# kornelski/cavif-rs

Hardware: AMD Instinct MI355X
Metric: MPix/s encoded at speed=4 q=80, 1080p batch; bit-exact vs CPU oracle (higher is better)
Workload: dtype u16 samples / i32 transform / i64 RD cost

## Files before the change

### cavif_rs_amd/csrc/dev_group.h

```cpp
#pragma once
#include "dev_predict.h"
#include "dev_txfm.h"
#include "dev_rate.h"

struct GroupBuf8 {
  int32_t tbuf[8 * 9];
  int32_t cbuf[64];
  int32_t qc[64];
  uint16_t rec[64];
  uint8_t lev[144];
};
#define GROUP_LANE (LANE & 15)
#define GROUP_ID (LANE >> 4)

template <int CTRL> __device__ __forceinline__ int dpp_row_(int v) { return __builtin_amdgcn_update_dpp(0, v, CTRL, 0xF, 0xF, false); }
__device__ __forceinline__ int row_sum_i32(int v) { v += dpp_row_<0x128>(v); v += dpp_row_<0x124>(v); v += dpp_row_<0x122>(v); v += dpp_row_<0x121>(v); return v; }
__device__ __forceinline__ int row_max_i32(int v) {
  v = imax_(v, dpp_row_<0x128>(v)); v = imax_(v, dpp_row_<0x124>(v)); v = imax_(v, dpp_row_<0x122>(v)); v = imax_(v, dpp_row_<0x121>(v)); return v;
}

static __device__ const int tx4_tab[2][3][4][8] = {
  { { { 2896, 2896, 2896, 2896, 0, 0, 0, 0 }, { 3784, 1567, -1567, -3784, 0, 0, 0, 0 }, { 2896, -2896, -2896, 2896, 0, 0, 0, 0 }, { 1567, -3784, 3784, -1567, 0, 0, 0, 0 } },
    { { 1321, 2482, 3344, 3803, 0, 0, 0, 0 }, { 3344, 3344, 0, -3344, 0, 0, 0, 0 }, { 3803, -1321, -3344, 2482, 0, 0, 0, 0 }, { 2482, -3803, 3344, -1321, 0, 0, 0, 0 } },
    { { 5793, 0, 0, 0, 0, 0, 0, 0 }, { 0, 5793, 0, 0, 0, 0, 0, 0 }, { 0, 0, 5793, 0, 0, 0, 0, 0 }, { 0, 0, 0, 5793, 0, 0, 0, 0 } } },
// ... 163 lines not shown
    int32_t x[N];
#pragma unroll
    for (int r = 0; r < N; r++) x[r] = (int32_t)((uint32_t)gb->tbuf[r * P + gl] << 2);
    tx1d<N>(x, ck, true);
#pragma unroll
    for (int r = 0; r < N; r++) gb->tbuf[r * P + gl] = N == 8 ? rshift_round_(x[r], 1) : x[r];
  }
  WAVE_SYNC();
  if (gl < N) {
    int32_t x[N];
#pragma unroll
    for (int c = 0; c < N; c++) x[c] = gb->tbuf[gl * P + c];
    tx1d<N>(x, rk, true);
#pragma unroll
    for (int c = 0; c < N; c++) gb->cbuf[gl * N + c] = x[c];
  }
  WAVE_SYNC();
  }
  const int dcq = f->dc_q[plane], acq = f->ac_q[plane];
  const uint32_t dc_recip = f->dc_recip[plane], ac_recip = f->ac_recip[plane];
  const int cls = tx_class_of(txtype), pt = plane > 0, txs_ctx = txs;
  const uint32_t dc_off = (uint32_t)(dcq * 109 / 256), off0 = (uint32_t)(acq * 98 / 256), off1 = (uint32_t)(acq * 109 / 256), off_eob = (uint32_t)(acq * 88 / 256);
  const uint32_t thr = (uint32_t)acq - off_eob, uq = (uint32_t)acq;
  int pos[IT]; uint32_t mag[IT]; int neg[IT];
  int last = 0;
#pragma unroll
  for (int k = 0; k < IT; k++) {
    const int i = gl + 16 * k;
    pos[k] = scan_pos(ls, N, cls, i);
    const int c = gb->cbuf[pos[k]];
    mag[k] = (uint32_t)iabs_(c); neg[k] = c < 0;
    if (i >= 1 && mag[k] >= thr) last = i + 1;
  }
  last = row_max_i32(last);
  const uint32_t x0 = (uint32_t)iabs_(gb->cbuf[0]) + dc_off;
  uint32_t l0u = __umulhi(x0, dc_recip);
  if (x0 - l0u * (uint32_t)dcq >= (uint32_t)dcq) l0u++;
  const int l0 = (int)l0u;
  int eob = last;
  if (eob == 0) eob = l0 ? 1 : 0;
  const int dmx = (1 << (7 + bd)) - 1, dmn = -(1 << (7 + bd));
  int lvl[IT];
  WAVE_SYNC();
#pragma unroll
  for (int k = 0; k < IT; k++) {
    const int i = gl + 16 * k;
    int lv = 0;
    if (i < eob) {
      if (i == 0) lv = l0;
      else {
        const uint32_t a = mag[k];
        uint32_t lv0 = __umulhi(a, ac_recip);
        if (a - lv0 * uq >= uq) lv0++;
        const uint32_t off = lv0 > 0 ? off1 : off0;
        lv = (int)lv0 + ((a + off) >= (lv0 + 1) * uq);
      }
    }
    lvl[k] = lv;
    const int pp = pos[k];
    gb->qc[pp] = neg[k] ? -lv : lv;
    gb->lev[(pp >> bwl) * st + (pp & (N - 1))] = (uint8_t)imin_(lv, 127);
    uint32_t m = (uint32_t)lv * (uint32_t)(pp == 0 ? dcq : acq);
    m &= 0xFFFFFF;
    const int v = neg[k] ? -(int)m : (int)m;
    gb->cbuf[pp] = v < dmn ? dmn : (v > dmx ? dmx : v);
  }
  WAVE_SYNC();
  uint32_t head = cc.txb[(txs_ctx * 13 + skip_ctx) * CDF_TXB_SKIP_STRIDE + (eob == 0)];
  int bits = 0, cul = 0, dcc = 0;
  if (eob > 0) {
    if (tx_off >= 0) head += tx_cost;
    const int eob_pt = eob_to_pt(eob);
    head += cc.eobpt[N == 4 ? 0 : 1][(pt * 2 + (cls == TXC_2D ? 0 : 1)) * (N == 4 ? CDF_EOB_PT_16_STRIDE : CDF_EOB_PT_64_STRIDE) + eob_pt - 1];
    if (eob_pt >= 3) {
      const int nb = eob_pt - 2, rem = eob - ((1 << (eob_pt - 2)) + 1), hi = (rem >> (nb - 1)) & 1;
      head += cc.eobx[((txs_ctx * 2 + pt) * 9 + (eob_pt - 3)) * CDF_EOB_EXTRA_STRIDE + hi];
      head += 512u * (uint32_t)(nb - 1);
    }
#pragma unroll
    for (int k = 0; k < IT; k++) {
      const int c = gl + 16 * k;
      if (c < eob) {
        const int pp = pos[k], row = pp >> bwl, col = pp & (N - 1), level = lvl[k];
        const LDS uint8_t *L = gb->lev + row * st + col;
        if (c == eob - 1) {
          const int ctx = c == 0 ? 0 : (c <= nc / 8 ? 1 : (c <= nc / 4 ? 2 : 3));
          bits += cc.beob[((txs_ctx * 2 + pt) * 4 + ctx) * CDF_COEFF_BASE_EOB_STRIDE + imin_(level, 3) - 1];
        } else {
          const int ctx = base_ctx(L, st, cls, row, col);
          bits += cc.base[((txs_ctx * 2 + pt) * 42 + ctx) * CDF_COEFF_BASE_STRIDE + imin_(level, 3)];
        }
        if (level > 2) {
          const int ctx = br_ctx(L, st, cls, row, col, c);
          const int off = ((imin_(txs_ctx, 3) * 2 + pt) * 21 + ctx) * CDF_COEFF_BR_STRIDE;
          int rem = level - 3;
          for (int idx = 0; idx < 4; idx++) { const int s2 = imin_(rem, 3); bits += cc.br[off + s2]; rem -= s2; if (s2 < 3) break; }
        }
        if (level) {
          if (c == 0) { bits += cc.dcs[(pt * 3 + dc_ctx) * CDF_DC_SIGN_STRIDE + neg[k]]; dcc = neg[k] ? 1 : 2; }
          else bits += 512;
          if (level > 14) { const int len = 32 - __clz(level - 14); bits += 512 * (2 * len - 1); }
        }
        cul += level;
      }
    }
  }
  bits = row_sum_i32(bits);
  const int cd = row_sum_i32(imin_(cul, 63) | (dcc << 16));
  res->eob = eob; res->cul = imin_(cd & 0xFFFF, 63); res->dcc = cd >> 16; res->rate = head + (uint32_t)bits;
  {
    constexpr int ROWSH = N == 4 ? 0 : 1;
    const int cbits = imax_(bd + 6, 16), cmax = (1 << (cbits - 1)) - 1, cmin = -(1 << (cbits - 1));
    if constexpr (N == 4) {
      if (eob > 0) {
        int v = iclamp_(tx4_inv(gb->cbuf[gl], rk), cmin, cmax);
        v = group_transpose4(v);
        t_rec = iclamp_(t_rec + round2_(tx4_inv(v, ck), 4), 0, (1 << bd) - 1);
        gb->rec[tidx] = (uint16_t)t_rec;
      }
      WAVE_SYNC();
    } else {
      const bool act = gl < N && eob > 0;
      if (act) {
        int32_t x[N];
  #pragma unroll
        for (int j = 0; j < N; j++) x[j] = gb->cbuf[gl * N + j];
        tx1d<N>(x, rk, false);
  #pragma unroll
        for (int j = 0; j < N; j++) gb->tbuf[gl * P + j] = iclamp_(round2_(x[j], ROWSH), cmin, cmax);
      }
      WAVE_SYNC();
      const int mx = (1 << bd) - 1;
      if (act) {
        int32_t x[N];
  #pragma unroll
        for (int i = 0; i < N; i++) x[i] = gb->tbuf[i * P + gl];
        tx1d<N>(x, ck, false);
  #pragma unroll
        for (int i = 0; i < N; i++) gb->rec[i * N + gl] = (uint16_t)iclamp_((int)gb->rec[i * N + gl] + round2_(x[i], 4), 0, mx);
      }
      WAVE_SYNC();
    }
  }
  int s = 0, sd = 0, qd = 0;
  if constexpr (N == 4) { const int d = t_src - t_rec; s = __mul24(d, d); sd = t_rec; qd = __mul24(t_rec, t_rec); }
  else
#pragma unroll
  for (int k = 0; k < IT; k++) { const int idx = gl + 16 * k; const int rv = gb->rec[idx], d = (int)src[idx] - rv; s += __mul24(d, d); sd += rv; qd += __mul24(rv, rv); }
  s = row_sum_i32(s);
  if (psy_sv >= 0) { sd = row_sum_i32(sd); qd = row_sum_i32(qd); res->sse = psy_cell_dist((uint32_t)s, (uint32_t)sd, (uint32_t)qd, (uint32_t)psy_sv, (uint32_t)psy_act, N == 4 ? 4 : 8, bd); }
  else res->sse = (int)(((unsigned long long)(uint32_t)s * (uint32_t)psy_act + 8192) >> 14);
}

struct GroupPredBuf { uint16_t wa[48], wl[48], tmp[32], pred[64]; };

__device__ __forceinline__ void edge_filter_group(LDS uint16_t *buf, int sz, int strength, LDS uint16_t *tmp, int gl) {
  if (strength) for (int i = gl; i < sz; i += 16) tmp[i] = buf[i - 1];
  WAVE_SYNC();
  if (strength) for (int i = 1 + gl; i < sz; i += 16) {
    int s = 0;
#pragma unroll
    for (int j = 0; j < 5; j++) {
      const int k = iclamp_(i - 2 + j, 0, sz - 1);
      const int kw = strength == 1 ? (j == 0 || j == 4 ? 0 : (j == 2 ? 8 : 4)) : (strength == 2 ? (j == 0 || j == 4 ? 0 : (j == 2 ? 6 : 5)) : (j == 0 || j == 4 ? 2 : 4));
      s += kw * tmp[k];
    }
    buf[i - 1] = (uint16_t)((s + 8) >> 4);
  }
  WAVE_SYNC();
}
__device__ __forceinline__ void edge_upsample_group(LDS uint16_t *buf, int num_px, int on, int bd, LDS uint16_t *tmp, int gl) {
  if (on) for (int i = gl; i < num_px + 3; i += 16) {
    uint16_t v;
    if (i == 0) v = buf[-1]; else if (i == num_px + 2) v = buf[num_px - 1]; else v = buf[i - 2];
    tmp[i] = v;
  }
  WAVE_SYNC();
  const int mx = (1 << bd) - 1;
  if (on) {
    if (gl == 0) buf[-2] = tmp[0];
    for (int i = gl; i < num_px; i += 16) {
      int s = -(int)tmp[i] + 9 * (int)tmp[i + 1] + 9 * (int)tmp[i + 2] - (int)tmp[i + 3];
      s = iclamp_(round2_(s, 4), 0, mx);
      buf[2 * i - 1] = (uint16_t)s;
      buf[2 * i] = tmp[i + 2];
    }
  }
  WAVE_SYNC();
}

template <int N>
__device__ inline void predict_dir_group(const LDS FrameDev *f, int x, int y, int have_left, int have_above, int pa, int ftype,
                                         const LDS uint16_t *ra, const LDS uint16_t *rl, LDS GroupPredBuf *gp, LDS uint16_t *out = nullptr) {
  constexpr int log2w = N == 4 ? 2 : 3, nn = N * N;
  const int gl = GROUP_LANE, bd = f->bd;
  const int max_x = f->mi_cols * 4 - 1, max_y = f->mi_rows * 4 - 1;
  LDS uint16_t *wa = gp->wa + EDGE_OFF, *wl = gp->wl + EDGE_OFF;
  for (int i = gl; i < 2 * N + 1; i += 16) { wa[i - 1] = ra[i - 1]; wl[i - 1] = rl[i - 1]; }
  WAVE_SYNC();
  const int diag = pa != 90 && pa != 180;
  {
    const int st_a = (diag && have_above) ? edge_strength_dev(N, N, ftype, pa - 90) : 0;
    const int num_a = imin_(N, max_x - x + 1) + (pa < 90 ? N : 0) + 1;
    edge_filter_group(wa, num_a, st_a, gp->tmp, gl);
    const int st_l = (diag && have_left) ? edge_strength_dev(N, N, ftype, pa - 180) : 0;
    const int num_l = imin_(N, max_y - y + 1) + (pa > 180 ? N : 0) + 1;
    edge_filter_group(wl, num_l, st_l, gp->tmp, gl);
  }
  const int up_a = edge_upsample_sel_dev(N, N, ftype, pa - 90);
  edge_upsample_group(wa, N + (pa < 90 ? N : 0), up_a, bd, gp->tmp, gl);
  const int up_l = edge_upsample_sel_dev(N, N, ftype, pa - 180);
  edge_upsample_group(wl, N + (pa > 180 ? N : 0), up_l, bd, gp->tmp, gl);
  int dx = 0, dy = 0;
  if (pa < 90) dx = dr_deriv_dev(pa); else if (pa > 90 && pa < 180) dx = dr_deriv_dev(180 - pa);
  if (pa > 90 && pa < 180) dy = dr_deriv_dev(pa - 90); else if (pa > 180) dy = dr_deriv_dev(270 - pa);
  for (int idx = gl; idx < nn; idx += 16) {
    const int i = idx >> log2w, j = idx & (N - 1);
    int v;
    if (pa < 90) {
      const int max_base = (2 * N - 1) << up_a;
      const int id = (i + 1) * dx, base = (id >> (6 - up_a)) + (j << up_a), sh = ((id << up_a) >> 1) & 0x1F;
      v = base < max_base ? round2_(wa[base] * (32 - sh) + wa[base + 1] * sh, 5) : wa[max_base];
    } else if (pa > 90 && pa < 180) {
      int id = (j << 6) - (i + 1) * dx, base = id >> (6 - up_a);
      if (base >= -(1 << up_a)) { const int sh = ((id << up_a) >> 1) & 0x1F; v = round2_(wa[base] * (32 - sh) + wa[base + 1] * sh, 5); }
      else { id = (i << 6) - (j + 1) * dy; base = id >> (6 - up_l); const int sh = ((id << up_l) >> 1) & 0x1F; v = round2_(wl[base] * (32 - sh) + wl[base + 1] * sh, 5); }
    } else if (pa > 180) {
      const int id = (j + 1) * dy, base = (id >> (6 - up_l)) + (i << up_l), sh = ((id << up_l) >> 1) & 0x1F;
      v = round2_(wl[base] * (32 - sh) + wl[base + 1] * sh, 5);
    } else if (pa == 90) v = wa[j];
    else v = wl[i];
    (out ? out : (LDS uint16_t *)gp->pred)[idx] = (uint16_t)v;
  }
  WAVE_SYNC();
}

template <int N>
__device__ inline void predict_nondir_group(int mode, int have_left, int have_above, int bd, const LDS uint16_t *ra, const LDS uint16_t *rl, LDS uint16_t *pred) {
  constexpr int log2w = N == 4 ? 2 : 3, IT = N * N / 16;
  constexpr unsigned long long wt = N == 4 ? 0x405595FFULL : 0x202532496992C5FFULL;
  const int gl = GROUP_LANE;
  if (mode == DC_PRED) {
    int v = 1 << (bd - 1);
    if (have_left || have_above) {
      int s = gl < N ? (have_above ? (int)ra[gl] : 0) + (have_left ? (int)rl[gl] : 0) : 0;
      s = row_sum_i32(s);
      v = (have_left && have_above) ? (s + N) >> (log2w + 1) : (s + (N >> 1)) >> log2w;
    }
#pragma unroll
    for (int k = 0; k < IT; k++) pred[gl + 16 * k] = (uint16_t)v;
  } else if (mode == PAETH_PRED) {
    const int tl = ra[-1];
#pragma unroll
    for (int k = 0; k < IT; k++) {
      const int idx = gl + 16 * k, i = idx >> log2w, j = idx & (N - 1);
      const int a = ra[j], l = rl[i], base = a + l - tl;
      const int pl = iabs_(base - l), pt = iabs_(base - a), ptl = iabs_(base - tl);
      pred[idx] = (uint16_t)((pl <= pt && pl <= ptl) ? l : (pt <= ptl ? a : tl));
    }
  } else if (mode >= 0) {
    const int bl = rl[N - 1], tr = ra[N - 1];
#pragma unroll
    for (int k = 0; k < IT; k++) {
      const int idx = gl + 16 * k, i = idx >> log2w, j = idx & (N - 1);
      const int wi = lut8(wt, i), wj = lut8(wt, j);
      const int vt = wi * (int)ra[j] + (256 - wi) * bl, ht = wj * (int)rl[i] + (256 - wj) * tr;
      pred[idx] = (uint16_t)(mode == SMOOTH_PRED ? round2_(vt + ht, 9) : round2_(mode == SMOOTH_V_PRED ? vt : ht, 8));
    }
  }
  WAVE_SYNC();
}

__device__ __forceinline__ int satd8_lane(int d0, int d1, int d2, int d3);
template <int N> __device__ inline int satd_group(const LDS uint16_t *src, const LDS uint16_t *pred) {
  constexpr int units = N * (N / 4);
  const int u = GROUP_LANE;
  if constexpr (N == 8) {
    const int xx = (u & 3) + ((u >> 1) & 4), o = (u & 4) * N + xx;
    const int d0 = (int)src[o] - (int)pred[o], d1 = (int)src[o + N] - (int)pred[o + N];
    const int d2 = (int)src[o + 2 * N] - (int)pred[o + 2 * N], d3 = (int)src[o + 3 * N] - (int)pred[o + 3 * N];
    return (row_sum_i32(satd8_lane(d0, d1, d2, d3)) + 2) >> 2;
  }
  int s = 0;
  if (u < units) {
    const int xx = u % N, o = (u / N) * 4 * N + xx;
    const int d0 = (int)src[o] - (int)pred[o], d1 = (int)src[o + N] - (int)pred[o + N];
    const int d2 = (int)src[o + 2 * N] - (int)pred[o + 2 * N], d3 = (int)src[o + 3 * N] - (int)pred[o + 3 * N];
    const int a = d0 + d1, b = d0 - d1, c = d2 + d3, e = d2 - d3;
    int t[4] = { a + c, b + e, a - c, b - e };
#pragma unroll
    for (int i = 0; i < 4; i++) {
      int v = __builtin_amdgcn_update_dpp(0, t[i], 0xB1, 0xF, 0xF, false);
      v = (LANE & 1) ? v - t[i] : t[i] + v;
      int w2 = __builtin_amdgcn_update_dpp(0, v, 0x4E, 0xF, 0xF, false);
      v = (LANE & 2) ? w2 - v : v + w2;
      s += iabs_(v);
    }
  }
  return row_sum_i32(s);
}
```

### cavif_rs_amd/csrc/tile_search.h

```cpp
#pragma once
#include "dev_common.h"
#include "dev_predict.h"
#include "dev_txfm.h"
#include "dev_rate.h"
#include "dev_group.h"

#ifndef MI_BALLOT64
#define MI_BALLOT64(p) __builtin_amdgcn_ballot_w64(p)
#endif
#define MI_K1_TRY_ATTR __attribute__((noinline, not_tail_called))
#define MI_K1_WG_PER_CU 4
#define WAVE_ID ((int)(threadIdx.x >> 6))
#ifndef MI_PROFILE
#define MI_PROFILE 0
#endif
#ifndef MI_PROF_MAXN
#define MI_PROF_MAXN 16
#endif
#ifndef MI_DEBUG_HOOKS
#define MI_DEBUG_HOOKS 0
#endif
#if MI_DEBUG_HOOKS
#define DBG_IS(f, v) ((f)->dbg == (v))
#else
// ... 485 lines not shown
  for (int e = W; e < ncand * ntx; e += NW) {
    const int ci = e / ntx, ti = e - ci * ntx, m = SH->order[ci];
    const int directional = m >= V_PRED && m <= D67_PRED;
    int delta = 0;
    const LDS uint16_t *lpred = S->pred;
    if (pred_cached) { delta = SH->ldelta[ci]; lpred = SH->lpred + ci * nn; }
    else {
      if (directional && refine) {
        long long bsd = SH->satd[m];
        for (int q = 0; q < 6; q++) { const long long sd = SH->dsd[ci][q]; if (sd < bsd) { bsd = sd; delta = dl_of(q); } }
      }
      predict_block(f, x, y, log2w, availL, availU, m, delta, ftype_y, ra, rl, wa, wl, S->etmp, S->pred);
    }
    const uint32_t mode_rate = y_mode_rate(k.cost(), ycost, m, directional && BS >= BS_8, delta);
    int ns2, set2;
    const int tx_off = intra_tx_cdf_r(f, Tools<TS>::reduced_tx_set(f), BS, m, &ns2, &set2);
    int txtype;
    if (ntx > 1) txtype = sym_to_txtype(tx_set, ti);
    else { txtype = mode_to_txtype(m); if (tx_off < 0 || txtype_to_sym(tx_set, txtype) < 0) txtype = DCT_DCT; }
    TxRes tr;
    long long j = eval_tx<MAXN, BS, NW>(k, 0, sctx_y, dctx_y, lpred, txtype, tx_off, tx_off >= 0 ? txtype_to_sym(tx_set, txtype) : 0, S->rec[cur], S->qc[cur], &tr);
    j += ((long long)mode_rate * f->rdmult + 256) >> 9;
    if (j < my_j) {
      my_j = j; my_e = e; my_mode = m; my_delta = delta; my_tx = txtype; my_tr = tr; my_mrate = mode_rate;
      cur ^= 1;
    }
  }
  if (LANE == 0) { SH->wbest_j[W] = my_j; SH->wbest_e[W] = my_e; }
  PH(6);
  WG_SYNC();
  PH(2);
  int win = 0;
  for (int w2 = 1; w2 < NW; w2++) if (SH->wbest_j[w2] < SH->wbest_j[win] || (SH->wbest_j[w2] == SH->wbest_j[win] && SH->wbest_e[w2] < SH->wbest_e[win])) win = w2;
  const long long best_j = SH->wbest_j[win];
  if (W == win) {
    const int b = cur ^ 1;
    const LDS uint16_t *best_rec = S->rec[b]; const LDS int32_t *best_qc = S->qc[b];
    if constexpr (SMALL_GROUPED) if (grouped) {
      if (parked) { best_rec = (const LDS uint16_t *)S->dcp; best_qc = (const LDS int32_t *)(S->dcp + 64); }
      else { best_rec = S->grp[my_g].rec; best_qc = S->grp[my_g].qc; }
    }
    commit_plane<BS>(f, 0, r, c, best_rec, best_qc, my_tr.eob, my_tr.cul, my_tr.dcc);
    fill_map_dev(f->m_ymode, ms, r, c, n4, my_mode);
    fill_map_dev((uint8_t *)f->m_angle_y, ms, r, c, n4, (uint8_t)(int8_t)my_delta);
    fill_map_dev(f->m_txtype, ms, r, c, n4, my_tr.eob ? my_tx : DCT_DCT);
    fill_map_dev(f->m_bsize, ms, r, c, n4, BS);
    fill_map_dev(f->m_txsize, ms, r, c, n4, BS);
    if (f->np > 1) for (int i = LANE; i < nn; i += 64) SH->luma_rec[i] = best_rec[i];
    if (LANE == 0) {
      SH->lm_mode = my_mode; SH->lm_delta = my_delta; SH->lm_tx = my_tx; SH->lm_eob = my_tr.eob;
      SH->lm_mode_j = ((long long)my_mrate * f->rdmult + 256) >> 9;
    }
  }
  PH(7);
  WG_SYNC();
  PH(2);
  if (DBG_IS(f, 5)) return 0;
  const int best_mode = SH->lm_mode, best_delta = SH->lm_delta;
  long long luma_j = best_j; int any_coef = SH->lm_eob > 0;
  if constexpr (BS > 0) if (Tools<TS>::tx_mode_select(f)) {
    const int maxw = 4 << BS;
    const int actx = nb_txU >= 0 && (1 << dim_wl(nb_txU)) >= maxw, lctx = nb_txL >= 0 && (1 << dim_hl(nb_txL)) >= maxw;
    const uint16_t *dcost = k.cost() + CDF_TX_SIZE + ((BS - 1) * 3 + actx + lctx) * CDF_TX_SIZE_STRIDE;
    luma_j += ((long long)dcost[0] * f->rdmult + 256) >> 9;
    if (tx_trial) {
      LDS int *const sub_tx = (LDS int *)SH->dsd, *const sub_eob = sub_tx + 16, *const sub_cul = sub_tx + 32, *const sub_dcc = sub_tx + 48, *const psv16 = sub_tx + 64;
      LDS int *const sfl_r = (LDS int *)SH->satd, *const sfl_b = sfl_r + 4;
      LDS uint16_t *ssrc = (LDS uint16_t *)SH->ssrc;
      auto trial = [&](auto depth_c) -> bool {
        constexpr int D = decltype(depth_c)::value;
        constexpr int SBS = BS - D, G = 1 << D, hn = n >> D, half = n4 >> D, hnn = hn * hn, SCS = hn < 32 ? hn : 32, sqn = SCS * SCS;
        long long j_split = SH->lm_mode_j + (((long long)dcost[D] * f->rdmult + 256) >> 9);
        int stx_ns = 0, stx_set = 0;
        const int stx_off = intra_tx_cdf_r(f, Tools<TS>::reduced_tx_set(f), SBS, best_mode, &stx_ns, &stx_set);
        const int sntx = stx_off >= 0 ? stx_ns : 1;
        int sub_any = 0;
#if MI_PROFILE
        const unsigned long long tr_t0_ = clock64();
        auto tr_done_ = [&]() { if (LANE == 0) SH->prof[W][BS == 1 ? 31 : (D == 1 ? 29 : 30)] += clock64() - tr_t0_; };
#else
        auto tr_done_ = []() {};
#endif
        PH(13);
        for (int q = W; q < G * G; q += NW) {
          const int so = (q / G) * hn * n + (q % G) * hn;
          for (int idx = LANE; idx < hnn; idx += 64) ssrc[q * hnn + idx] = SH->srcb[0][so + (idx / hn) * n + (idx % hn)];
        }
        if (W == 0) {
          if (LANE < n4) {
            const int k2 = LANE;
            const bool ha = availU && c + k2 < f->mi_cols, hl = availL && r + k2 < f->mi_rows;
            const int ia = ha ? (r - 1) * ms + c + k2 : mi, il = hl ? (r + k2) * ms + c - 1 : mi;
            const int la = f->m_lvl[0][ia], da = f->m_dc[0][ia], ll = f->m_lvl[0][il], dl2 = f->m_dc[0][il];
            SH->nb_top[k2][0] = (uint8_t)(ha ? la : 0); SH->nb_top[k2][1] = (uint8_t)(ha ? da : 0);
            SH->nb_left[k2][0] = (uint8_t)(hl ? ll : 0); SH->nb_left[k2][1] = (uint8_t)(hl ? dl2 : 0);
          }
          if (hn == 4 && n == 16 && LANE < 16) psv16[LANE] = (int)f->svar4[(r + (LANE >> 2)) * ms + c + (LANE & 3)];
          if (LANE >= 1 && LANE < G) {
            const bool ca = c + n4 < t->mi_col_end, cb = r + n4 < t->mi_row_end;
            sfl_r[LANE] = ca && decoded_before(r, c, 0, r + LANE * half - 1, c + n4); sfl_b[LANE] = cb && decoded_before(r, c, 0, r + n4, c + LANE * half - 1);
          }
        }
        WG_SYNC();
        PH(22);
        [[maybe_unused]] const int x_ = x, y_ = y, r_ = r, c_ = c, availU_ = availU, availL_ = availL, have_ar_ = have_ar, have_bl_ = have_bl, best_mode_ = best_mode, best_delta_ = best_delta, ftype_y_ = ftype_y;
        if constexpr (SBS <= BS_8 && NW == 4 && MAXN <= 32) {
          constexpr int CH_BYTES = nn * 2 + G * G * sqn * 4 + G * G * 4;
          static_assert(4 * CH_BYTES <= (int)sizeof(WaveScratch<MAXN>) && hnn <= 64 && 4 * 64 <= MAXN * MAXN, "four chains fit a wavefront's scratch; edges and predictions of four rows fit pred / dcp");
          const int g = GROUP_ID, gl = GROUP_LANE;
          const bool paired = MAXN == 16 && sntx == 5 && n >= 8 && hn <= 8;
          const int mem = paired ? (g & 1) : 0;
          const int e = paired ? (W == 0 ? 1 + (g >> 1) : (W == 1 ? 3 + (g >> 1) : ((W == 2 && g < 2) ? 0 : 64)))
                               : (sntx == 5 ? (W == 0 ? g + 1 : ((W == 1 && g == 0) ? 0 : 64)) : W * 4 + g);
          const bool has_chain = e < sntx, wave_has = paired ? W < 3 : (sntx == 5 ? W < 2 : W * 4 < sntx);
          LDS long long *const cres_j = (LDS long long *)SH->cj;
          LDS int *const cres_any = (LDS int *)(cres_j + 8);
          LDS uint32_t *const meta_idtx = (LDS uint32_t *)SH->cj + 32;
          const long long thr = uni64(luma_j < budget ? luma_j : budget);
          auto chain_state = [&](int ce, int cw, int cg, LDS uint16_t **cv, LDS int32_t **cq, LDS uint32_t **cm) {
            if (paired && ce == 0) { *cv = split_rec; *cq = split_qc; *cm = meta_idtx; return; }
            LDS uint8_t *cst = paired ? (LDS uint8_t *)k.wave(3) + (ce >= 1 && ce <= 4 ? ce - 1 : 0) * CH_BYTES : (LDS uint8_t *)k.wave(2 + cw) + cg * CH_BYTES;
            *cv = (LDS uint16_t *)cst; *cq = (LDS int32_t *)(cst + nn * 2); *cm = (LDS uint32_t *)(cst + nn * 2 + G * G * sqn * 4);
          };
          if (wave_has) {
            const int x = uni32(x_), y = uni32(y_), r = uni32(r_), c = uni32(c_), availU = uni32(availU_), availL = uni32(availL_), have_ar = uni32(have_ar_), have_bl = uni32(have_bl_);
            const int best_mode = uni32(best_mode_), best_delta = uni32(best_delta_), ftype_y = uni32(ftype_y_);
            LDS uint16_t *canvas; LDS int32_t *cqc; LDS uint32_t *cmeta;
            chain_state(e, W, g, &canvas, &cqc, &cmeta);
            LDS uint16_t *A = S->pred + g * 64 + EDGE_OFF, *Lf = A + 32, *ppred = S->dcp + g * 64;
            int txtype;
            if (sntx > 1) txtype = sym_to_txtype(stx_set, has_chain ? e : 0);
            else { txtype = mode_to_txtype(best_mode); if (stx_off < 0 || txtype_to_sym(stx_set, txtype) < 0) txtype = DCT_DCT; }
            const int tx_sym = stx_off >= 0 ? txtype_to_sym(stx_set, txtype) : 0;
            const bool dirm = best_mode >= V_PRED && best_mode <= D67_PRED;
            const int pa = dirm ? mode_angle_of(best_mode) + 3 * best_delta : 0;
            const int max_x = f->mi_cols * 4 - 1, max_y = f->mi_rows * 4 - 1, rs = f->stride, bd = f->bd;
            const uint16_t *grec = f->rec[0];
            long long jc = has_chain ? j_split : J_INF;
            int any = 0;
            const bool uses_ar = dirm && pa < 90;
            const int nslot = paired ? (G == 4 ? 10 : (uses_ar ? 4 : 3)) : G * G;
#pragma unroll 1
            for (int slot = 0; slot < nslot; slot++) {
              if (MI_BALLOT64(jc < thr) == 0ull) break;
              int q0 = slot, q1 = -1;
              if (paired) {
                if (G == 4) { const int lo = imax_(0, (slot - 2) >> 1), hi = imin_(3, slot >> 1); q0 = lo * 4 + slot - 2 * lo; q1 = lo + 1 <= hi ? (lo + 1) * 4 + slot - 2 * (lo + 1) : -1; }
                else if (!uses_ar) { q0 = slot == 0 ? 0 : (slot == 1 ? 1 : 3); q1 = slot == 1 ? 2 : -1; }
              }
              const int q = (mem == 1 && q1 >= 0) ? q1 : q0;
              const int bi = q / G, bj = q % G;
              const int sx = x + bj * hn, sy = y + bi * hn;
              const int sU = availU || bi, sL = availL || bj;
              {
                const int s_ar = bi == 0 ? (bj < G - 1 ? availU : have_ar) : (bj < G - 1 ? 1 : sfl_r[bi]);
                const int s_bl = bj == 0 ? (bi < G - 1 ? availL : have_bl) : (bi < G - 1 ? 0 : sfl_b[bj]);
                const int lim_a = imin_(max_x, sx + (s_ar ? 2 * hn : hn) - 1), lim_l = imin_(max_y, sy + (s_bl ? 2 * hn : hn) - 1);
                auto px = [&](int ax, int ay) -> int {
                  const int xr = ax - x, yr = ay - y;
                  const bool in_blk = xr >= 0 && xr < n && yr >= 0 && yr < n, on_a = yr == -1 && xr >= -1 && xr < 2 * n, on_l = xr == -1 && yr >= 0 && yr < 2 * n;
                  const LDS uint16_t *p = in_blk ? (const LDS uint16_t *)canvas + (yr * n + xr) : (on_a ? ra + xr : rl + (on_l ? yr : 0));
                  int v = (int)*p;
                  if (!(in_blk || on_a || on_l)) v = (int)grec[(size_t)ay * rs + ax];
                  return v;
                };
#pragma unroll
                for (int it = 0; it < (2 * hn + 16) / 16; it++) {
                  const int i = gl + 16 * it;
                  const bool act = i <= 2 * hn, corner = i == 2 * hn;
                  const int ii = act ? i : 0;
                  int a, l;
                  if (sU) a = px(corner ? (sL ? sx - 1 : sx) : imin_(lim_a, sx + ii), sy - 1); else a = px(sL ? sx - 1 : sx, sy);
                  if (sL) l = px(sx - 1, imin_(lim_l, sy + ii)); else l = px(sx, sU ? sy - 1 : sy);
                  if (!sU && !sL) { a = corner ? (1 << (bd - 1)) : (1 << (bd - 1)) - 1; l = (1 << (bd - 1)) + 1; }
                  if (act && corner) { A[-1] = (uint16_t)a; Lf[-1] = (uint16_t)a; }
                  if (act && !corner) { A[ii] = (uint16_t)a; Lf[ii] = (uint16_t)l; }
                }
              }
              WAVE_SYNC();
              if (dirm) predict_dir_group<hn>(f, sx, sy, sL, sU, pa, ftype_y, A, Lf, &S->gpred[g], ppred);
              else predict_nondir_group<hn>(best_mode, sL, sU, bd, A, Lf, ppred);
              PH(23);
              int ssc, sdc;
              {
                int top = 0, left = 0, dcs = 0;
                const uint32_t mt = bi ? cmeta[q - G] : 0u, ml = bj ? cmeta[q - 1] : 0u;
#pragma unroll
                for (int k2 = 0; k2 < half; k2++) {
                  int l, d;
                  if (bi == 0) { l = SH->nb_top[bj * half + k2][0]; d = SH->nb_top[bj * half + k2][1]; } else { l = (int)((mt >> 16) & 0xFF); d = (int)(mt >> 24); if (n >= 32 && c + bj * half + k2 >= f->mi_cols) l = d = 0; }
                  top = imax_(top, l); dcs += d == 1 ? -1 : (d == 2 ? 1 : 0);
                  if (bj == 0) { l = SH->nb_left[bi * half + k2][0]; d = SH->nb_left[bi * half + k2][1]; } else { l = (int)((ml >> 16) & 0xFF); d = (int)(ml >> 24); if (n >= 32 && r + bi * half + k2 >= f->mi_rows) l = d = 0; }
                  left = imax_(left, l); dcs += d == 1 ? -1 : (d == 2 ? 1 : 0);
                }
                sdc = dcs < 0 ? 1 : (dcs > 0 ? 2 : 0);
                if (top == 0 && left == 0) ssc = 1;
                else if (top == 0 || left == 0) ssc = 2 + (imax_(top, left) > 3);
                else if (imax_(top, left) <= 3) ssc = 4;
                else if (imin_(top, left) <= 3) ssc = 5;
                else ssc = 6;
              }
              constexpr int pcp = n >= 8 ? n / 8 : 1;
              const int psv_q = hn == 4 ? (n == 8 ? SH->psv4[q] : psv16[q]) : SH->psv[bi * pcp + bj];
              const int pact_q = hn == 4 ? SH->pact[(bi >> 1) * pcp + (bj >> 1)] : SH->pact[bi * pcp + bj];
              GroupRes gr;
              eval_group<hn>(k.cc(), k.cost(), k.ls(), f, &S->grp[g], ssrc + q * hnn, ppred, 0, SBS, txtype, ssc, sdc, stx_off, tx_sym, Tools<TS>::tune_psnr(f) ? -1 : psv_q, pact_q, &gr);
              {
                const long long j = rd_dist32(f, 0, gr.sse) + rd_rate32(f, gr.rate);
                long long jslot = j;
                if (paired) {
                  const long long jo = ((long long)__shfl((int)(j >> 32), LANE ^ 16) << 32) | (unsigned int)__shfl((int)j, LANE ^ 16);
                  jslot = q1 >= 0 ? j + jo : (mem == 0 ? j : jo);
                }
                if (has_chain) jc += jslot;
              }
              if (has_chain) {
                const LDS uint16_t *srec = S->grp[g].rec; const LDS int32_t *sqc = S->grp[g].qc;
                const int ro = bi * hn * n + bj * hn;
#pragma unroll
                for (int i = gl; i < hnn; i += 16) canvas[ro + (i / hn) * n + (i % hn)] = srec[i];
#pragma unroll
                for (int i = gl; i < sqn; i += 16) cqc[q * sqn + i] = sqc[i];
                cmeta[q] = (uint32_t)gr.eob | ((uint32_t)gr.cul << 16) | ((uint32_t)gr.dcc << 24);
              }
              any |= gr.eob > 0;
              WAVE_SYNC();
              PH(25);
            }
            if (paired) any |= __shfl(any, LANE ^ 16);
            const int rslot = paired ? (has_chain ? e : 5 + (g & 1)) : (sntx == 5 ? (W == 0 ? g + 1 : (g == 0 ? 0 : 4 + g)) : W * 4 + g);
            cres_j[rslot] = (has_chain && jc < thr) ? jc : J_INF; cres_any[rslot] = any;
          }
          __builtin_amdgcn_s_setprio(0);
          WG_SYNC();
          PH(26);
          int be = -1; long long bjc = J_INF;
          for (int e2 = 0; e2 < sntx; e2++) { const long long v = cres_j[e2]; if (v < bjc) { bjc = v; be = e2; } }
          j_split = bjc;
          if (be >= 0) {
            const int ow = paired ? 0 : (sntx == 5 ? (be == 0 ? 1 : 0) : be >> 2), og = sntx == 5 ? (be == 0 ? 0 : be - 1) : be & 3;
            if (W == ow) {
              LDS uint16_t *canvas; LDS int32_t *cqc; LDS uint32_t *cmeta;
              chain_state(be, ow, og, &canvas, &cqc, &cmeta);
              if (canvas != split_rec) {
                for (int i = LANE; i < nn; i += 64) split_rec[i] = canvas[i];
                for (int i = LANE; i < G * G * sqn; i += 64) split_qc[i] = cqc[i];
              }
              int btx;
              if (sntx > 1) btx = sym_to_txtype(stx_set, be);
              else { btx = mode_to_txtype(best_mode); if (stx_off < 0 || txtype_to_sym(stx_set, btx) < 0) btx = DCT_DCT; }
              if (LANE < G * G) { const uint32_t m = cmeta[LANE]; const int eob = (int)(m & 0xFFFF); sub_eob[LANE] = eob; sub_cul[LANE] = (int)((m >> 16) & 0xFF); sub_dcc[LANE] = (int)(m >> 24); sub_tx[LANE] = eob ? btx : DCT_DCT; }
            }
            sub_any = cres_any[be];
            WG_SYNC();
          }
          PH(27);
        } else {
          static_assert(nn <= (int)(sizeof(S->rec[1]) / 2) && G * G * sqn <= (int)(sizeof(S->qc[1]) / 4) && G * G <= 16, "a chain's state fits the wave's second candidate buffers");
          LDS uint16_t *canvas = S->rec[1]; LDS int32_t *cqc = S->qc[1]; LDS uint32_t *cmeta = (LDS uint32_t *)SH->cj + W * 16;
          LDS uint16_t *A = S->pred + EDGE_OFF, *Lf = S->pred + (MAXN * MAXN / 2) + EDGE_OFF;
          LDS int *ppsv = (LDS int *)S->etmp, *ppact = ppsv + 16;
          static_assert(sizeof(S->etmp) >= 32 * sizeof(int), "the sub-block's psychovisual references fit etmp");
          const int max_x = f->mi_cols * 4 - 1, max_y = f->mi_rows * 4 - 1, rs = f->stride, bd = f->bd;
          const uint16_t *grec = f->rec[0];
          const long long j0 = j_split;
          long long best_chain = J_INF;
          sub_any = 0;
#pragma unroll 1
          for (int rd = 0; rd * NW < sntx; rd++) {
            const int e = rd * NW + W;
            const bool has_chain = e < sntx;
            long long thr = luma_j < budget ? luma_j : budget;
            if (best_chain < thr) thr = best_chain;
            int txtype;
            if (sntx > 1) txtype = sym_to_txtype(stx_set, has_chain ? e : 0);
            else { txtype = mode_to_txtype(best_mode); if (stx_off < 0 || txtype_to_sym(stx_set, txtype) < 0) txtype = DCT_DCT; }
            const int tx_sym = stx_off >= 0 ? txtype_to_sym(stx_set, txtype) : 0;
            long long jc = has_chain ? j0 : J_INF;
            int any = 0;
            if (has_chain) {
#pragma unroll 1
              for (int q = 0; q < G * G; q++) {
                if (!(jc < thr)) break;
                const int bi = q / G, bj = q % G;
                const int sx = x + bj * hn, sy = y + bi * hn;
                const int sU = availU || bi, sL = availL || bj;
                {
                  const int s_ar = bi == 0 ? (bj < G - 1 ? availU : have_ar) : (bj < G - 1 ? 1 : sfl_r[bi]);
                  const int s_bl = bj == 0 ? (bi < G - 1 ? availL : have_bl) : (bi < G - 1 ? 0 : sfl_b[bj]);
                  const int lim_a = imin_(max_x, sx + (s_ar ? 2 * hn : hn) - 1), lim_l = imin_(max_y, sy + (s_bl ? 2 * hn : hn) - 1);
                  auto px = [&](int ax, int ay) -> int {
                    const int xr = ax - x, yr = ay - y;
                    if (xr >= 0 && xr < n && yr >= 0 && yr < n) return (int)canvas[yr * n + xr];
                    if (yr == -1 && xr >= -1 && xr < 2 * n) return (int)ra[xr];
                    if (xr == -1 && yr >= 0 && yr < 2 * n) return (int)rl[yr];
                    return (int)grec[(size_t)ay * rs + ax];
                  };
                  for (int i = LANE; i <= 2 * hn; i += 64) {
                    const bool corner = i == 2 * hn;
                    int a, l;
                    if (sU) a = px(corner ? (sL ? sx - 1 : sx) : imin_(lim_a, sx + i), sy - 1); else a = px(sL ? sx - 1 : sx, sy);
                    if (sL) l = px(sx - 1, imin_(lim_l, sy + i)); else l = px(sx, sU ? sy - 1 : sy);
                    if (!sU && !sL) { a = corner ? (1 << (bd - 1)) : (1 << (bd - 1)) - 1; l = (1 << (bd - 1)) + 1; }
                    if (corner) { A[-1] = (uint16_t)a; Lf[-1] = (uint16_t)a; } else { A[i] = (uint16_t)a; Lf[i] = (uint16_t)l; }
                  }
                  WAVE_SYNC();
                  predict_block(f, sx, sy, log2w - D, sL, sU, best_mode, best_delta, ftype_y, A, Lf, wa, wl, S->etmp, S->dcp);
                }
                PH(23);
                int ssc, sdc;
                {
                  int top = 0, left = 0, dcs = 0;
                  const uint32_t mt = bi ? cmeta[q - G] : 0u, ml = bj ? cmeta[q - 1] : 0u;
#pragma unroll
                  for (int k2 = 0; k2 < half; k2++) {
                    int l, d;
                    if (bi == 0) { l = SH->nb_top[bj * half + k2][0]; d = SH->nb_top[bj * half + k2][1]; } else { l = (int)((mt >> 16) & 0xFF); d = (int)(mt >> 24); if (n >= 32 && c + bj * half + k2 >= f->mi_cols) l = d = 0; }
                    top = imax_(top, l); dcs += d == 1 ? -1 : (d == 2 ? 1 : 0);
                    if (bj == 0) { l = SH->nb_left[bi * half + k2][0]; d = SH->nb_left[bi * half + k2][1]; } else { l = (int)((ml >> 16) & 0xFF); d = (int)(ml >> 24); if (n >= 32 && r + bi * half + k2 >= f->mi_rows) l = d = 0; }
                    left = imax_(left, l); dcs += d == 1 ? -1 : (d == 2 ? 1 : 0);
                  }
                  sdc = dcs < 0 ? 1 : (dcs > 0 ? 2 : 0);
                  if (top == 0 && left == 0) ssc = 1;
                  else if (top == 0 || left == 0) ssc = 2 + (imax_(top, left) > 3);
                  else if (imax_(top, left) <= 3) ssc = 4;
                  else if (imin_(top, left) <= 3) ssc = 5;
                  else ssc = 6;
                }
                constexpr int pcp = n >= 8 ? n / 8 : 1, scp = hn >= 8 ? hn / 8 : 1;
                if (LANE < scp * scp) {
                  if constexpr (hn == 4) { ppsv[0] = n == 8 ? SH->psv4[q] : psv16[q]; ppact[0] = SH->pact[(bi >> 1) * pcp + (bj >> 1)]; }
                  else { const int pc = (bi * scp + LANE / scp) * pcp + bj * scp + LANE % scp; ppsv[LANE] = SH->psv[pc]; ppact[LANE] = SH->pact[pc]; }
                }
                WAVE_SYNC();
// ... 877 lines not shown
```

Before: 544.3.

## Keep directional-prediction edges in registers and filter them with DPP row shuffles

```diff
diff --git a/cavif_rs_amd/csrc/dev_group.h b/cavif_rs_amd/csrc/dev_group.h
--- a/cavif_rs_amd/csrc/dev_group.h
+++ b/cavif_rs_amd/csrc/dev_group.h
@@ -339,65 +339,62 @@
   else res->sse = (int)(((unsigned long long)(uint32_t)s * (uint32_t)psy_act + 8192) >> 14);
 }
 
-struct GroupPredBuf { uint16_t wa[48], wl[48], tmp[32], pred[64]; };
-
-__device__ __forceinline__ void edge_filter_group(LDS uint16_t *buf, int sz, int strength, LDS uint16_t *tmp, int gl) {
-  if (strength) for (int i = gl; i < sz; i += 16) tmp[i] = buf[i - 1];
-  WAVE_SYNC();
-  if (strength) for (int i = 1 + gl; i < sz; i += 16) {
-    int s = 0;
-#pragma unroll
-    for (int j = 0; j < 5; j++) {
-      const int k = iclamp_(i - 2 + j, 0, sz - 1);
-      const int kw = strength == 1 ? (j == 0 || j == 4 ? 0 : (j == 2 ? 8 : 4)) : (strength == 2 ? (j == 0 || j == 4 ? 0 : (j == 2 ? 6 : 5)) : (j == 0 || j == 4 ? 2 : 4));
-      s += kw * tmp[k];
-    }
-    buf[i - 1] = (uint16_t)((s + 8) >> 4);
-  }
-  WAVE_SYNC();
-}
-__device__ __forceinline__ void edge_upsample_group(LDS uint16_t *buf, int num_px, int on, int bd, LDS uint16_t *tmp, int gl) {
-  if (on) for (int i = gl; i < num_px + 3; i += 16) {
-    uint16_t v;
-    if (i == 0) v = buf[-1]; else if (i == num_px + 2) v = buf[num_px - 1]; else v = buf[i - 2];
-    tmp[i] = v;
-  }
-  WAVE_SYNC();
-  const int mx = (1 << bd) - 1;
-  if (on) {
-    if (gl == 0) buf[-2] = tmp[0];
-    for (int i = gl; i < num_px; i += 16) {
-      int s = -(int)tmp[i] + 9 * (int)tmp[i + 1] + 9 * (int)tmp[i + 2] - (int)tmp[i + 3];
-      s = iclamp_(round2_(s, 4), 0, mx);
-      buf[2 * i - 1] = (uint16_t)s;
-      buf[2 * i] = tmp[i + 2];
-    }
-  }
-  WAVE_SYNC();
-}
+struct GroupPredBuf { uint16_t wa[48], wl[48], pred[64]; };
+
+#ifndef MI_BALLOT64
+#define MI_BALLOT64(p) __builtin_amdgcn_ballot_w64(p)
+#endif
+template <int CTRL> __device__ __forceinline__ int dpp_row_f(int fill, int v) { return __builtin_amdgcn_update_dpp(fill, v, CTRL, 0xF, 0xF, false); }
 
 template <int N>
-__device__ inline void predict_dir_group(const LDS FrameDev *f, int x, int y, int have_left, int have_above, int pa, int ftype,
-                                         const LDS uint16_t *ra, const LDS uint16_t *rl, LDS GroupPredBuf *gp, LDS uint16_t *out = nullptr) {
+__device__ __forceinline__ void edge_filter_row(int &t, int &hi, int sz, int strength, int gl) {
+  const int r0 = strength == 3 ? 2 : 0, r1 = strength == 0 ? 0 : (strength == 2 ? 5 : 4);
+  const bool act = gl >= 1 && gl < sz;
+  const int k0 = act ? r0 : 0, k1 = act ? r1 : 0;
+  const int m1 = dpp_row_f<0x111>(t, t), m2 = dpp_row_f<0x112>(t, t), p1 = dpp_row_f<0x101>(hi, t), p2 = dpp_row_f<0x102>(hi, t);
+  const int m2c = gl >= 2 ? m2 : m1;
+  const int p1c = gl + 1 < sz ? p1 : t, p2c = gl + 2 < sz ? p2 : p1c;
+  if constexpr (N == 8) {
+    const int h0 = sz == 17 ? r0 : 0, h1 = sz == 17 ? r1 : 0;
+    const int x14 = gl == 15 ? m1 : t, x15 = gl == 15 ? t : p1;
+    hi = (h0 * x14 + h1 * x15 + (16 - h0 - h1) * hi + 8) >> 4;
+  }
+  t = (k0 * (m2c + p2c) + k1 * (m1 + p1c) + (16 - 2 * k0 - 2 * k1) * t + 8) >> 4;
+}
+template <int N>
+__device__ __forceinline__ void edge_store_row(LDS uint16_t *buf, int t, int hi, int num_px, int on, int any_on, int bd, int gl) {
+  int s = 0, p1 = 0;
+  if (any_on) {
+    const int m1 = dpp_row_f<0x111>(t, t); p1 = dpp_row_f<0x101>(hi, t); const int p2 = dpp_row_f<0x102>(hi, t);
+    const int m1c = gl >= 1 ? m1 : t, p2c = gl + 2 <= num_px ? p2 : p1;
+    s = iclamp_(round2_(-m1c + 9 * t + 9 * p1 - p2c, 4), 0, (1 << bd) - 1);
+  }
+  const bool up = on != 0, body = up ? gl < num_px : gl < 2 * N + 1;
+  const bool last = up ? gl == num_px - 1 : (N == 8 && gl == 15);
+  if (body) buf[up ? 2 * gl - 2 : gl - 1] = (uint16_t)t;
+  if (up && body) buf[2 * gl - 1] = (uint16_t)s;
+  if (last) buf[up ? 2 * gl : 15] = (uint16_t)(up ? p1 : hi);
+}
+
+template <int N>
+__device__ inline void predict_dir_group_r(const LDS FrameDev *f, int x, int y, int have_left, int have_above, int pa, int ftype,
+                                           int ta, int tl, int ha, int hl, LDS GroupPredBuf *gp, LDS uint16_t *out = nullptr) {
   constexpr int log2w = N == 4 ? 2 : 3, nn = N * N;
   const int gl = GROUP_LANE, bd = f->bd;
   const int max_x = f->mi_cols * 4 - 1, max_y = f->mi_rows * 4 - 1;
   LDS uint16_t *wa = gp->wa + EDGE_OFF, *wl = gp->wl + EDGE_OFF;
-  for (int i = gl; i < 2 * N + 1; i += 16) { wa[i - 1] = ra[i - 1]; wl[i - 1] = rl[i - 1]; }
-  WAVE_SYNC();
   const int diag = pa != 90 && pa != 180;
-  {
-    const int st_a = (diag && have_above) ? edge_strength_dev(N, N, ftype, pa - 90) : 0;
-    const int num_a = imin_(N, max_x - x + 1) + (pa < 90 ? N : 0) + 1;
-    edge_filter_group(wa, num_a, st_a, gp->tmp, gl);
-    const int st_l = (diag && have_left) ? edge_strength_dev(N, N, ftype, pa - 180) : 0;
-    const int num_l = imin_(N, max_y - y + 1) + (pa > 180 ? N : 0) + 1;
-    edge_filter_group(wl, num_l, st_l, gp->tmp, gl);
-  }
-  const int up_a = edge_upsample_sel_dev(N, N, ftype, pa - 90);
-  edge_upsample_group(wa, N + (pa < 90 ? N : 0), up_a, bd, gp->tmp, gl);
-  const int up_l = edge_upsample_sel_dev(N, N, ftype, pa - 180);
-  edge_upsample_group(wl, N + (pa > 180 ? N : 0), up_l, bd, gp->tmp, gl);
+  const int st_a = (diag && have_above) ? edge_strength_dev(N, N, ftype, pa - 90) : 0;
+  const int st_l = (diag && have_left) ? edge_strength_dev(N, N, ftype, pa - 180) : 0;
+  const int up_a = edge_upsample_sel_dev(N, N, ftype, pa - 90), up_l = edge_upsample_sel_dev(N, N, ftype, pa - 180);
+  if (MI_BALLOT64((st_a | st_l) != 0) != 0ull) {
+    edge_filter_row<N>(ta, ha, imin_(N, max_x - x + 1) + (pa < 90 ? N : 0) + 1, st_a, gl);
+    edge_filter_row<N>(tl, hl, imin_(N, max_y - y + 1) + (pa > 180 ? N : 0) + 1, st_l, gl);
+  }
+  const int any_up = MI_BALLOT64((up_a | up_l) != 0) != 0ull;
+  edge_store_row<N>(wa, ta, ha, N + (pa < 90 ? N : 0), up_a, any_up, bd, gl);
+  edge_store_row<N>(wl, tl, hl, N + (pa > 180 ? N : 0), up_l, any_up, bd, gl);
+  WAVE_SYNC();
   int dx = 0, dy = 0;
   if (pa < 90) dx = dr_deriv_dev(pa); else if (pa > 90 && pa < 180) dx = dr_deriv_dev(180 - pa);
   if (pa > 90 && pa < 180) dy = dr_deriv_dev(pa - 90); else if (pa > 180) dy = dr_deriv_dev(270 - pa);
@@ -423,6 +420,13 @@
 }
 
 template <int N>
+__device__ inline void predict_dir_group(const LDS FrameDev *f, int x, int y, int have_left, int have_above, int pa, int ftype,
+                                         const LDS uint16_t *ra, const LDS uint16_t *rl, LDS GroupPredBuf *gp, LDS uint16_t *out = nullptr) {
+  const int gl = GROUP_LANE, i = imin_(gl, 2 * N) - 1;
+  predict_dir_group_r<N>(f, x, y, have_left, have_above, pa, ftype, ra[i], rl[i], N == 8 ? ra[15] : 0, N == 8 ? rl[15] : 0, gp, out);
+}
+
+template <int N>
 __device__ inline void predict_nondir_group(int mode, int have_left, int have_above, int bd, const LDS uint16_t *ra, const LDS uint16_t *rl, LDS uint16_t *pred) {
   constexpr int log2w = N == 4 ? 2 : 3, IT = N * N / 16;
   constexpr unsigned long long wt = N == 4 ? 0x405595FFULL : 0x202532496992C5FFULL;
diff --git a/cavif_rs_amd/csrc/tile_search.h b/cavif_rs_amd/csrc/tile_search.h
--- a/cavif_rs_amd/csrc/tile_search.h
+++ b/cavif_rs_amd/csrc/tile_search.h
@@ -661,34 +661,37 @@
               const int bi = q / G, bj = q % G;
               const int sx = x + bj * hn, sy = y + bi * hn;
               const int sU = availU || bi, sL = availL || bj;
+              int ea, el, eha = 0, ehl = 0;
               {
                 const int s_ar = bi == 0 ? (bj < G - 1 ? availU : have_ar) : (bj < G - 1 ? 1 : sfl_r[bi]);
                 const int s_bl = bj == 0 ? (bi < G - 1 ? availL : have_bl) : (bi < G - 1 ? 0 : sfl_b[bj]);
                 const int lim_a = imin_(max_x, sx + (s_ar ? 2 * hn : hn) - 1), lim_l = imin_(max_y, sy + (s_bl ? 2 * hn : hn) - 1);
-                auto px = [&](int ax, int ay) -> int {
-                  const int xr = ax - x, yr = ay - y;
-                  const bool in_blk = xr >= 0 && xr < n && yr >= 0 && yr < n, on_a = yr == -1 && xr >= -1 && xr < 2 * n, on_l = xr == -1 && yr >= 0 && yr < 2 * n;
-                  const LDS uint16_t *p = in_blk ? (const LDS uint16_t *)canvas + (yr * n + xr) : (on_a ? ra + xr : rl + (on_l ? yr : 0));
-                  int v = (int)*p;
-                  if (!(in_blk || on_a || on_l)) v = (int)grec[(size_t)ay * rs + ax];
-                  return v;
+                const int ya = bi * hn - 1, xl = bj * hn - 1;
+                const LDS uint16_t *pa_ = !sU ? (bj ? (const LDS uint16_t *)canvas + xl : rl) : (bi ? (const LDS uint16_t *)canvas + ya * n + bj * hn : ra + bj * hn);
+                const LDS uint16_t *pl_ = !sL ? (bi ? (const LDS uint16_t *)canvas + ya * n : ra) : (bj ? (const LDS uint16_t *)canvas + bi * hn * n + xl : rl + bi * hn);
+                const LDS uint16_t *pc_ = !sU ? pa_ : ((bi && !bj && sL) ? rl + ya : pa_ - (sL ? 1 : 0));
+                const int ca = sU ? lim_a - sx : 0, cl = sL ? lim_l - sy : 0, sl_ = sL ? (bj ? n : 1) : 0;
+                const bool ga = sU && bi, gb = sL && bj;
+                const int flat = (!sU && !sL) ? (1 << (bd - 1)) : 0;
+                auto edge = [&](int ii, bool corner, int &a, int &l) {
+                  const int ia = imin_(ii, ca), il = imin_(ii, cl);
+                  const bool fa = ga && !corner && bj * hn + ia >= n, fl = gb && bi * hn + il >= n;
+                  a = (int)*(corner ? pc_ : pa_ + (fa ? 0 : ia)); l = (int)pl_[fl ? 0 : il * sl_];
+                  if (fa) a = (int)grec[(size_t)(sy - 1) * rs + sx + ia];
+                  if (fl) l = (int)grec[(size_t)(sy + il) * rs + sx - 1];
+                  if (flat) { a = corner ? flat : flat - 1; l = flat + 1; }
                 };
-#pragma unroll
-                for (int it = 0; it < (2 * hn + 16) / 16; it++) {
-                  const int i = gl + 16 * it;
-                  const bool act = i <= 2 * hn, corner = i == 2 * hn;
-                  const int ii = act ? i : 0;
-                  int a, l;
-                  if (sU) a = px(corner ? (sL ? sx - 1 : sx) : imin_(lim_a, sx + ii), sy - 1); else a = px(sL ? sx - 1 : sx, sy);
-                  if (sL) l = px(sx - 1, imin_(lim_l, sy + ii)); else l = px(sx, sU ? sy - 1 : sy);
-                  if (!sU && !sL) { a = corner ? (1 << (bd - 1)) : (1 << (bd - 1)) - 1; l = (1 << (bd - 1)) + 1; }
-                  if (act && corner) { A[-1] = (uint16_t)a; Lf[-1] = (uint16_t)a; }
-                  if (act && !corner) { A[ii] = (uint16_t)a; Lf[ii] = (uint16_t)l; }
-                }
+                edge(imin_(imax_(gl - 1, 0), 2 * hn - 1), gl == 0, ea, el);
+                if (gl == 0) el = ea;
+                if constexpr (hn == 8) edge(15, false, eha, ehl);
               }
-              WAVE_SYNC();
-              if (dirm) predict_dir_group<hn>(f, sx, sy, sL, sU, pa, ftype_y, A, Lf, &S->gpred[g], ppred);
-              else predict_nondir_group<hn>(best_mode, sL, sU, bd, A, Lf, ppred);
+              if (dirm) predict_dir_group_r<hn>(f, sx, sy, sL, sU, pa, ftype_y, ea, el, eha, ehl, &S->gpred[g], ppred);
+              else {
+                if (gl <= 2 * hn) { A[gl - 1] = (uint16_t)ea; Lf[gl - 1] = (uint16_t)el; }
+                if (hn == 8 && gl == 15) { A[15] = (uint16_t)eha; Lf[15] = (uint16_t)ehl; }
+                WAVE_SYNC();
+                predict_nondir_group<hn>(best_mode, sL, sU, bd, A, Lf, ppred);
+              }
               PH(23);
               int ssc, sdc;
               {
```

Result: no change. 544.5, median of 5 (+0.0%).
